# LoganWilliams1/mhm2_kmer_analysis_v2

Hardware: AMD Instinct MI355X
Metric: k-mers/sec (kcount stage) at k=21 (higher is better)
Workload: dtype u64

## Files before the change

### mhm2_kmer_analysis_v2_amd/csrc/kc_api.hip

```cpp
#include <hip/hip_runtime.h>

#include <math.h>
#include <stdio.h>
#include <stdlib.h>
#include <string.h>

#include <algorithm>
#include <new>
#include <thread>
#include <type_traits>
#include <vector>

#include "../../include/kcount_mi355.h"
#include "kc_bucketed.hpp"
#include "kc_shard.hpp"
#include "kc_wire6.hpp"
#include "kc_supermer.hpp"
#include "kc_ctg.hpp"

using namespace kc;

static thread_local char g_last_error[512] = "";

static int hip_fail(hipError_t e, const char *what, int line) {
// ... 630 lines not shown
  int rc = KC_OK;
  for (int i = 0; i < NCAND && !rc; i++) {
    rate[i] = probe(cand[i], wpw);
    const double gib = probe(cand[i], wpw_gib);
    if (rate[i] < 0 || gib <= 0) rc = KC_ERR_HIP;
    else ratio[i] = rate[i] / gib;
    if (log) fprintf(stderr, "kc arena probe (%s): allocation %d, %.2f TB/s, %.2f of its first GiB alone, %p\n", what, i, rate[i], ratio[i], (void *)cand[i]);
    if (rc || ratio[i] >= KC_ARENA_OK || i == NCAND - 1) break;
    size_t free_b = 0, total_b = 0;
    if (hipMemGetInfo(&free_b, &total_b) != hipSuccess || free_b < bytes + ((size_t)8 << 30)) break;
    if (hipMalloc((void **)&cand[i + 1], bytes) != hipSuccess) {
      (void)hipGetLastError();
      cand[i + 1] = nullptr;
      break;
    }
    ncand = i + 2;
  }
  int best_i = -1;
  for (int i = 0; i < ncand; i++)
    if (cand[i] && (best_i < 0 || ratio[i] > ratio[best_i])) best_i = i;
  for (int i = 0; i < ncand; i++)
    if (i != best_i && cand[i]) (void)hipFree(cand[i]);
  *arena = best_i >= 0 ? cand[best_i] : nullptr;
  c->arena_probe_tbps = best_i >= 0 ? rate[best_i] : 0.0;
  (void)hipEventDestroy(e0);
  (void)hipEventDestroy(e1);
  if (!rc && !*arena) rc = KC_ERR_OUT_OF_MEMORY;
  if (rc) snprintf(g_last_error, sizeof(g_last_error), "choosing the %s arena failed", what);
  return rc;
}

constexpr double KC_MAX_REGION_LOAD = 0.72;

static int bk_init(kc_ctx *c) {
  if (c->bk_ready) return KC_OK;
  const kc_tuning &t = c->tuning;
  Geom &g = c->gm;
  memset(&g, 0, sizeof(g));
  const uint64_t bcap = c->cfg.max_kmers_buffered ? c->cfg.max_kmers_buffered : (1ULL << 26);
  double est = c->cfg.max_elems ? (double)c->cfg.max_elems : 0.35 * (double)bcap;
  const double flow_n = ((c->cfg.flags & KC_FLAG_SHARD_BUCKETS) && c->cfg.rank_n > 1) ? (double)c->cfg.rank_n : 1.0;
  est *= flow_n;
  const uint32_t smax = count_smax(c->nl);
  g.S = t.slots ? std::min(std::max(t.slots, 16u), smax) : smax;
  while (g.S & (g.S - 1)) g.S &= g.S - 1;
  const double target_load = 0.4;
  if (!t.slots && est <= KC_MAX_REGION_LOAD * (double)(1u << 20) * (g.S / 2)) g.S /= 2;
  const uint64_t regions_needed = std::min<uint64_t>((uint64_t)(est / (target_load * g.S)) + 1, 1ULL << 20);
  g.P1 = t.p1 ? t.p1 : (uint32_t)std::max<double>(1.0, floor(sqrt((double)regions_needed)));
  g.P2 = t.p2 ? t.p2 : (uint32_t)((regions_needed + g.P1 - 1) / g.P1);
  if (c->nl == 1 && c->k <= KC_COMPACT_MAX_K && t.mode != 2) {
    uint32_t la = 0, lb = 0;
    if (t.p1 || t.p2) {
      la = ilog2(g.P1);
      lb = ilog2(g.P2);
    } else {
      const uint32_t lr = std::min<uint32_t>(20, ilog2(regions_needed));
      la = lr / 2;
      lb = lr - la;
      if (2u * (uint32_t)c->k + 6u <= 32u + lr && la >= 1) {
        g.P1 = 1u << la;
        g.P2 = 1u << lb;
      }
    }
    if (g.P1 == (1u << la) && g.P2 == (1u << lb) && la >= 1 && lb >= 1 && 2u * (uint32_t)c->k + 6u <= 32u + la + lb &&
        2u * (uint32_t)c->k > la + lb) {
      g.cp = 1;
      g.la = la;
      g.lb = lb;
      g.k2 = 2u * (uint32_t)c->k;
    }
  }
  if (g.P1 < 1 || g.P2 < 1 || g.P1 > PMAX || g.P2 > PMAX) return KC_ERR_INVALID_ARG;
  g.rec6 = (c->nl == 1 && g.cp && g.k2 - g.la <= 32) ? 1u : 0u;
  c->wire6 = (c->cfg.flags & KC_FLAG_WIRE_UNITS) && g.rec6 && g.k2 - g.la - g.lb >= 21 && !(c->cfg.flags & KC_FLAG_REFERENCE_OWNER) &&
             c->cfg.rank_n >= 1 && c->cfg.rank_n <= (int)WIRE6_MAX_SHARDS;
  g.G = t.writers ? std::min<uint32_t>(t.writers, GMAX)
                  : (uint32_t)std::max<uint64_t>(1, std::min<uint64_t>((uint64_t)std::min<int>(c->num_cus, GMAX), bcap / (4 * 16384)));
  if (g.G < 1) g.G = 1;
  const uint64_t R = (uint64_t)g.P1 * g.P2;
  const double mean1 = (double)bcap / ((double)g.G * g.P1), mean2 = flow_n * (double)bcap / (double)R;
  g.log2CH1 = t.chunk1 ? ilog2(t.chunk1) : std::min<uint32_t>(12, std::max<uint32_t>(4, ilog2((uint64_t)(mean1 / 8) + 1)));
  g.log2CH2 = t.chunk2 ? ilog2(t.chunk2) : std::min<uint32_t>(10, std::max<uint32_t>(4, ilog2((uint64_t)(mean2 / 8) + 1)));
  const uint64_t CH1 = 1ULL << g.log2CH1, CH2 = 1ULL << g.log2CH2;
  g.L1MAX = t.chain1_max ? t.chain1_max : (uint32_t)(4.0 * mean1 / (double)CH1) + 8;
  g.L2MAX = std::min<uint32_t>(CHAIN_LDS, t.chain2_max ? t.chain2_max : (uint32_t)(4.0 * mean2 / (double)CH2) + 8);
  if (g.cp && !t.chain2_max) g.L2MAX = std::min<uint32_t>(CHAIN_LDS, std::max<uint32_t>(g.L2MAX, (uint32_t)((KC_COUNT_MAX + CH2) / CH2) + 1));
  g.A1 = t.arena1 ? t.arena1 : (uint32_t)(1.03 * (double)bcap / ((double)g.G * (double)CH1)) + g.P1 + 16;
  const uint64_t a2 = bcap / CH2 + R + g.P1 + 16;
  if (a2 >= (1ULL << 32) || (uint64_t)g.A1 * g.G >= (1ULL << 32) || bcap / g.P1 >= (1ULL << 31)) return KC_ERR_INVALID_ARG;
  g.A2 = (uint32_t)a2;
  BucketBufs &b = c->bb;
  memset(&b, 0, sizeof(b));
  b.ovf1_cap = t.ovf_capacity ? t.ovf_capacity : std::max<uint64_t>(bcap / (c->nl == 1 ? 4 : 8) + 4096, 2 * (uint64_t)SUPER_SPAN);
  b.ovf2_cap = t.ovf_capacity ? t.ovf_capacity : std::max<uint64_t>(bcap / (c->nl == 1 ? 32 : 64) + 4096, 2 * (uint64_t)SUPER_SPAN);
  const size_t w = (size_t)c->nl * 8;
  const size_t nseg = (size_t)g.G * g.P1;
  const size_t rec1_bytes = (size_t)g.G * g.A1 * CH1 * (g.rec6 ? 6 : w) + 64, rec2_bytes = (size_t)g.A2 * CH2 * (g.cp ? 4 : w);
  bool rec1_reused = false, rec2_reused = false;
  {
    int rc = bk_take(c, 0, (void **)&b.rec1, rec1_bytes, &rec1_reused);
    const char *pe = getenv("KC_ARENA_PROBE");
    if (!rc && !(pe && pe[0] == '0') && rec1_bytes >= ((size_t)1 << 30) && !rec1_reused) {
      rc = pick_fast_arena(c, &b.rec1, rec1_bytes, g.G, "level 1");
    }
    if (!rc) rc = bk_take(c, 1, (void **)&b.chain1, nseg * g.L1MAX * 4);
    if (!rc) rc = bk_take(c, 2, (void **)&b.cnt1, nseg * 4);
    if (!rc) rc = bk_take(c, 3, (void **)&b.used1, (size_t)g.G * 2 * 4);
    if (!rc) rc = bk_take(c, 4, (void **)&b.rec2, rec2_bytes, &rec2_reused);
    if (!rc) rc = bk_take(c, 5, (void **)&b.chain2, (size_t)R * g.L2MAX * 4);
    if (!rc) rc = bk_take(c, 6, (void **)&b.cnt2, (size_t)R * 4);
    if (!rc) rc = bk_take(c, 7, (void **)&b.base2, ((size_t)g.P1 + 1) * 4);
    if (!rc) rc = bk_take(c, 8, (void **)&b.flag, (size_t)R * 4);
    if (!rc) rc = bk_take(c, 9, (void **)&b.ovf1, b.ovf1_cap * w);
    if (!rc) rc = bk_take(c, 10, (void **)&b.ovf2, b.ovf2_cap * w);
    if (!rc) rc = bk_take(c, 11, (void **)&b.done1, nseg * 4);
    if (!rc) rc = bk_take(c, 12, (void **)&b.used2, (size_t)g.P1 * 4);
    if (rc) return rc;
  }
  c->inc_on = false;
  c->l2_per_bucket = 0;
  HIPCHK(hipMemsetAsync(b.cnt1, 0, nseg * 4, c->stream));
  HIPCHK(hipMemsetAsync(b.used1, 0, (size_t)g.G * 2 * 4, c->stream));
  HIPCHK(hipMemsetAsync(b.cnt2, 0, (size_t)R * 4, c->stream));
  HIPCHK(hipMemsetAsync(b.flag, 0, (size_t)R * 4, c->stream));
  HIPCHK(hipMemsetAsync(c->d_cb, 0, CB_COUNT * 8, c->stream));
  if (getenv("KC_DEBUG_ADDR"))
    fprintf(stderr, "kc arenas: rec1 %p (%zu MB) chain1 %p cnt1 %p rec2 %p chain2 %p ovf1 %p ovf2 %p\n", (void *)b.rec1, rec1_bytes >> 20,
            (void *)b.chain1, (void *)b.cnt1, (void *)b.rec2, (void *)b.chain2, (void *)b.ovf1, (void *)b.ovf2);
  c->bk_bytes = rec1_bytes + rec2_bytes + (b.ovf1_cap + b.ovf2_cap) * w + nseg * (g.L1MAX + 1) * 4 + (size_t)R * (g.L2MAX + 2) * 4;
  c->bk_capacity = bcap;
  c->bk_ready = true;
  c->bk_level2 = c->bk_flagged = false;
  c->bk_rot = 0;
  return KC_OK;
}

static int sync_cb(kc_ctx *c) {
  HIPCHK(hipMemcpyAsync(c->h_cb, c->d_cb, CB_COUNT * 8, hipMemcpyDeviceToHost, c->stream));
  HIPCHK(hipStreamSynchronize(c->stream));
  return KC_OK;
}

static int bk_ovf1_room(kc_ctx *c, uint64_t want, uint64_t *room) {
  if (c->ovf1_ub + want <= c->bb.ovf1_cap) {
    *room = c->bb.ovf1_cap - c->ovf1_ub;
    return KC_OK;
  }
  int rc = sync_cb(c);
  if (rc) return rc;
  if (c->h_cb[CB_FATAL] & ~(c->inc_on ? (uint64_t)FATAL_OVF2 : 0ULL)) {
    snprintf(g_last_error, sizeof(g_last_error), "k-mer buffer: records were lost (fatal bits %llu)", (unsigned long long)c->h_cb[CB_FATAL]);
    return KC_ERR_CAPACITY;
  }
  uint64_t used = std::min<uint64_t>(c->h_cb[CB_OVF1], c->bb.ovf1_cap);
  if (used && c->bb.ovf1_cap - used < want && !c->sh.extracting) {
    rc = ensure_room(c, used);
    if (rc) return rc;
    {
      KernelTimer kt(c, KT_FALLBACK);
      with_nl(c, [&](auto nl) {
        auto kern = with_cp<nl>(c, [&](auto cp) { return kc_ovf1_drain_kernel<nl, cp>; });
        hipLaunchKernelGGL(kern, dim3((unsigned)std::min<uint64_t>((used + TPB - 1) / TPB, 256 * 32)), dim3(TPB), 0, c->stream, c->gm, c->bb,
                           used, c->table, c->d_ctrs);
      });
    }
// ... 1297 lines not shown
  *owner = (int)shard_of_bucket(b1, c->gm.P1, (uint32_t)c->cfg.rank_n);
  return KC_OK;
}

extern "C" int kc_flush(kc_ctx *c) {
  if (!c) return KC_ERR_INVALID_ARG;
  HIPCHK(hipSetDevice(c->cfg.device));
  int rc = sync_ctrs(c);
  if (rc) return rc;
  if (c->h_ctrs[CTR_BAD_BASE]) return KC_ERR_BAD_BASE;
  return KC_OK;
}

static int alloc_results(kc_ctx *c, uint64_t cap) {
  if (!cap) cap = 1;
  if (c->d_out_keys && c->out_cap >= cap) {
    c->out_n = 0;
    free_index(c);
    return KC_OK;
  }
  free_results(c);
  HIPCHK(hipMalloc((void **)&c->d_out_keys, cap * c->nl * 8));
  HIPCHK(hipMalloc((void **)&c->d_out_counts, cap * 2));
  HIPCHK(hipMalloc((void **)&c->d_out_left, cap));
  HIPCHK(hipMalloc((void **)&c->d_out_right, cap));
  c->out_cap = cap;
  return KC_OK;
}

static int grow_results(kc_ctx *c, uint64_t need, uint64_t keep) {
  if (need <= c->out_cap) return KC_OK;
  uint64_t *k0 = c->d_out_keys;
  uint16_t *c0 = c->d_out_counts;
  uint8_t *l0 = c->d_out_left, *r0 = c->d_out_right;
  c->d_out_keys = nullptr;
  c->d_out_counts = nullptr;
  c->d_out_left = c->d_out_right = nullptr;
  int rc = alloc_results(c, need);
  if (!rc && keep) {
    HIPCHK(hipMemcpyAsync(c->d_out_keys, k0, keep * c->nl * 8, hipMemcpyDeviceToDevice, c->stream));
    HIPCHK(hipMemcpyAsync(c->d_out_counts, c0, keep * 2, hipMemcpyDeviceToDevice, c->stream));
    HIPCHK(hipMemcpyAsync(c->d_out_left, l0, keep, hipMemcpyDeviceToDevice, c->stream));
    HIPCHK(hipMemcpyAsync(c->d_out_right, r0, keep, hipMemcpyDeviceToDevice, c->stream));
    HIPCHK(hipStreamSynchronize(c->stream));
  }
  if (k0) (void)hipFree(k0);
  if (c0) (void)hipFree(c0);
  if (l0) (void)hipFree(l0);
  if (r0) (void)hipFree(r0);
  return rc;
}

static int table_finalize_append(kc_ctx *c) {
  int rc = sync_ctrs(c);
  if (rc) return rc;
  const uint64_t entries = c->h_ctrs[CTR_ENTRIES];
  if (!entries) return KC_OK;
  rc = grow_results(c, c->h_ctrs[CTR_OUT] + entries, c->h_ctrs[CTR_OUT]);
  if (rc) return rc;
  {
    KernelTimer kt(c, KT_FINALIZE);
    const unsigned nblk = (unsigned)std::min<uint64_t>((c->capacity + TPB - 1) / TPB, 256 * 16);
    with_nl(c, [&](auto nl) {
      hipLaunchKernelGGL(kc_finalize_kernel<nl>, dim3(nblk), dim3(TPB), 0, c->stream, c->table, c->capacity, c->cfg.dmin_thres, c->d_out_keys,
                         c->d_out_counts, c->d_out_left, c->d_out_right, c->d_ctrs);
    });
  }
  HIPCHK(hipGetLastError());
  return KC_OK;
}

template <int NL>
static int bk_level2_launch(kc_ctx *c, bool inc) {
  const bool cr = use_cp<NL>(c) && c->gm.k2 - c->gm.la <= 32;
  const bool fl = shard_flow_only(c);
  if (inc && fl) return KC_ERR_STATE;
  auto kern = with_cp<NL>(c, [&](auto cp) {
    if (inc) return cr ? kc_l2_split_kernel<NL, cp, cp, false, true> : kc_l2_split_kernel<NL, cp, false, false, true>;
    if (cr) return fl ? kc_l2_split_kernel<NL, cp, cp, true> : kc_l2_split_kernel<NL, cp, cp, false>;
    return fl ? kc_l2_split_kernel<NL, cp, false, true> : kc_l2_split_kernel<NL, cp, false, false>;
  });
  const bool r6 = NL == 1 && c->gm.rec6 != 0;
  auto kern6 = inc ? kc_l2_rec6_kernel<false, true> : (fl ? kc_l2_rec6_kernel<true, false> : kc_l2_rec6_kernel<false, false>);
  int rc = r6 ? set_dyn_lds(kern6, l2r6_lds_bytes()) : set_dyn_lds(kern, lds_l2<NL>());
  if (rc) return rc;
  FlatSrc fs;
  memset(&fs, 0, sizeof(fs));
  fs.b_hi = c->gm.P1;
  if (fl) {
    fs.cnt = c->sh.d_cnt;
    fs.at = c->sh.d_at;
    fs.F = c->sh.F;
    fs.b_lo = shard_first_bucket((uint32_t)c->cfg.rank_me, c->gm.P1, (uint32_t)c->cfg.rank_n);
    fs.b_hi = shard_first_bucket((uint32_t)c->cfg.rank_me + 1, c->gm.P1, (uint32_t)c->cfg.rank_n);
    fs.nbo = fs.b_hi - fs.b_lo;
  }
  if (!inc || !c->inc_on) {
    if (inc && !c->l2_per_bucket) c->l2_per_bucket = (c->bk_capacity + c->gm.P1 - 1) / c->gm.P1;
    const uint64_t per_bucket = inc ? c->l2_per_bucket : 0;
    hipLaunchKernelGGL(kc_bucket_prefix_kernel, dim3(1), dim3(WGB), 0, c->stream, c->gm, c->bb, fs, c->d_cb, per_bucket);
    c->num_gpu_calls++;
    if (inc) {
      HIPCHK(hipMemsetAsync(c->bb.cnt2, 0, (size_t)c->gm.P1 * c->gm.P2 * 4, c->stream));
      HIPCHK(hipMemsetAsync(c->bb.done1, 0, (size_t)c->gm.G * c->gm.P1 * 4, c->stream));
      HIPCHK(hipMemsetAsync(c->bb.used2, 0, (size_t)c->gm.P1 * 4, c->stream));
      c->inc_on = true;
    }
  }
  if (fs.b_hi > fs.b_lo) {
    KernelTimer kt(c, r6 ? KT_L2_REC6 : KT_L2_SPLIT);
    const dim3 grid(std::min<unsigned>(fs.b_hi - fs.b_lo, (unsigned)c->num_cus));
    if (r6) hipLaunchKernelGGL(kern6, grid, dim3(WGB), l2r6_lds_bytes(), c->stream, c->gm, c->bb, fs, c->d_cb);
    else hipLaunchKernelGGL(kern, grid, dim3(WGB), lds_l2<NL>(), c->stream, c->gm, c->bb, fs, c->d_cb);
  }
  HIPCHK(hipGetLastError());
  return KC_OK;
}

static int bk_level2_instalment(kc_ctx *c) {
  if (!bk_active(c) || !c->bk_ready || c->bk_level2 || c->sh.flow) return KC_OK;
  return with_nl(c, [&](auto nl) { return bk_level2_launch<nl>(c, true); });
}

static int bk_l2_reserve(kc_ctx *c, uint64_t need) {
  const Geom &g = c->gm;
  const uint64_t CH2 = 1ULL << g.log2CH2;
  const uint64_t pb_need = (uint64_t)((double)need * 1.08 / (double)g.P1) + 2 * CH2;
  const uint64_t pb_now = c->inc_on ? c->l2_per_bucket : (c->bk_capacity + g.P1 - 1) / g.P1;
  if (pb_need <= pb_now) {
    if (!c->inc_on) c->l2_per_bucket = pb_now;
    return KC_OK;
  }
  const uint64_t pb = c->inc_on ? std::max<uint64_t>(2 * pb_now, pb_need) : pb_need;
  const uint64_t a2 = (uint64_t)g.P1 * ((pb + CH2 - 1) / CH2 + g.P2) + 16;
  if (a2 >= (1ULL << 32)) return KC_ERR_OUT_OF_MEMORY;
  uint64_t *bigger = nullptr;
  const size_t bytes = (size_t)a2 * CH2 * 4;
  size_t free_b = 0, total_b = 0;
  if (hipMemGetInfo(&free_b, &total_b) != hipSuccess || free_b < bytes + ((size_t)4 << 30) || hipMalloc((void **)&bigger, bytes) != hipSuccess) {
    (void)hipGetLastError();
    return KC_ERR_OUT_OF_MEMORY;
  }
  if (c->inc_on) {
    uint32_t *nb = nullptr;
    if (hipMalloc((void **)&nb, ((size_t)g.P1 + 1) * 4) != hipSuccess) {
      (void)hipGetLastError();
      (void)hipFree(bigger);
      return KC_ERR_OUT_OF_MEMORY;
    }
    BucketBufs tmp = c->bb;
    tmp.base2 = nb;
    FlatSrc fs;
    memset(&fs, 0, sizeof(fs));
    hipLaunchKernelGGL(kc_bucket_prefix_kernel, dim3(1), dim3(WGB), 0, c->stream, c->gm, tmp, fs, c->d_cb, pb);
    hipLaunchKernelGGL(kc_l2_grow_kernel, dim3(g.P1), dim3(WGB), 0, c->stream, c->gm, reinterpret_cast<const uint32_t *>(c->bb.rec2),
                       reinterpret_cast<uint32_t *>(bigger), c->bb.base2, nb, c->bb.used2, c->bb.chain2, c->bb.cnt2);
    c->num_gpu_calls += 2;
    hipError_t e = hipGetLastError();
    if (e == hipSuccess) e = hipMemcpyAsync(c->bb.base2, nb, ((size_t)g.P1 + 1) * 4, hipMemcpyDeviceToDevice, c->stream);
    if (e == hipSuccess) e = hipStreamSynchronize(c->stream);
    (void)hipFree(nb);
    if (e != hipSuccess) {
      (void)hipFree(bigger);
      return hip_fail(e, "bk_l2_reserve", __LINE__);
    }
  }
  HIPCHK(hipFree(c->bb.rec2));
  c->bk_bytes += bytes - c->bk_held[4];
  c->bb.rec2 = bigger;
  c->bk_held[4] = bytes;
  c->gm.A2 = (uint32_t)a2;
  c->l2_per_bucket = pb;
  return KC_OK;
}

static int l2_snapshot(kc_ctx *c) {
  const Geom &g = c->gm;
  const size_t b_cnt2 = (size_t)g.P1 * g.P2 * 4, b_used2 = (size_t)g.P1 * 4, b_done1 = (size_t)g.G * g.P1 * 4, need = b_cnt2 + b_used2 + b_done1 + 8;
  c->l2snap_fresh = !c->inc_on;
  if (c->l2snap_fresh) return KC_OK;
  if (c->l2snap_bytes < need) {
    if (c->d_l2snap) HIPCHK(hipFree(c->d_l2snap));
    c->d_l2snap = nullptr;
    c->l2snap_bytes = 0;
    HIPCHK(hipMalloc((void **)&c->d_l2snap, need));
    c->l2snap_bytes = need;
  }
  HIPCHK(hipMemcpyAsync(c->d_l2snap, c->bb.cnt2, b_cnt2, hipMemcpyDeviceToDevice, c->stream));
  HIPCHK(hipMemcpyAsync(c->d_l2snap + b_cnt2, c->bb.used2, b_used2, hipMemcpyDeviceToDevice, c->stream));
  HIPCHK(hipMemcpyAsync(c->d_l2snap + b_cnt2 + b_used2, c->bb.done1, b_done1, hipMemcpyDeviceToDevice, c->stream));
  HIPCHK(hipMemcpyAsync(c->d_l2snap + b_cnt2 + b_used2 + b_done1, c->d_cb + CB_OVF2, 8, hipMemcpyDeviceToDevice, c->stream));
  return KC_OK;
}
static int l2_restore_and_grow(kc_ctx *c, uint64_t need, uint64_t kept) {
  const Geom &g = c->gm;
// ... 925 lines not shown
```

### mhm2_kmer_analysis_v2_amd/csrc/kc_bucketed.hpp

```cpp
#pragma once
#include "kc_kernels.hpp"

namespace kc {

constexpr int WGB = 1024;
constexpr int SUPER_SPAN = 16 * WGB - PRE - POST;
using TileSuper = TileGeo<WGB, SUPER_SPAN>;
static_assert(TileSuper::GPT == 1 && TileSuper::NGROUP == WGB, "one group per thread");
constexpr int PMAX = 1024;
constexpr int GMAX = 512;

template <int NL> struct Rnd {
  static constexpr int RPOS = NL == 1 ? 16 : NL == 2 ? 8 : 4;
  static constexpr int RPOS_READS = NL == 1 ? 8 : NL <= 3 ? 4 : 2;
  static constexpr size_t STAGE = ((size_t)WGB * RPOS + 64) * NL * 8;
  static constexpr size_t STAGE_READS = ((size_t)WGB * RPOS_READS + 64) * NL * 8;
};

struct Geom {
  uint32_t G, P1, P2, S;
  uint32_t log2CH1, log2CH2;
  uint32_t L1MAX, L2MAX;
  uint32_t A1;
  uint32_t A2;
// ... 1219 lines not shown
          } else {
            lo[j] = (uint32_t)(nxt[j][0] >> (64u - gm.k2));
            ext = (uint32_t)nxt[j][0] & 63u;
          }
          br[j] = ((lo[j] >> sh_b2) & (P2 - 1u)) | (ext << 10);
        } else {
#pragma unroll
          for (int w = 0; w < NL; w++) rec[j][w] = nxt[j][w];
        }
      }
    };
    if (n) load_round(0);
    take_over();
    if (per_round < n) load_round(per_round);
    int buf = 0;
    for (uint32_t v0 = 0; v0 < n; v0 += per_round) {
#pragma unroll
      for (int j = 0; j < RPOS; j++) {
        const bool valid = v0 + (uint32_t)j * WGB + tid < n;
        uint32_t b;
        if constexpr (CR) b = br[j] & (PMAX - 1);
        else b = CP ? cp_b2(rec[j][0], gm) : hash_b2(rec_hash<NL>(rec[j]), gm);
        const uint32_t rank = hist_rank(L.sp, buf, b, valid);
        if constexpr (CR) br[j] = valid ? (br[j] | (rank << 16)) : ~0u;
        else br[j] = valid ? (b | (rank << 10)) : ~0u;
      }
      KC_SPLIT_STAMP(0)
      lds_barrier();
      const uint32_t total = split_stage<NL, RPOS, CR ? 16 : 10>(
          L.sp, sorted, nullptr, buf, P2,
          [&](int j, uint64_t (&o)[NL]) {
            if constexpr (CR) {
              o[0] = ((uint64_t)b1 << (64u - gm.la)) | ((uint64_t)lo[j] << (64u - gm.k2)) | (uint64_t)((br[j] >> 10) & 63u);
            } else {
#pragma unroll
              for (int w = 0; w < NL; w++) o[w] = rec[j][w];
            }
          },
          br, D, cst);
      take_over();
      if (v0 + 2 * (uint64_t)per_round < n) load_round(v0 + 2 * per_round);
      KC_SPLIT_STAMP(5)
      split_copy_out<NL>(
          L.sp, sorted, nullptr, total, D, [&](const uint64_t (&r)[NL]) { return CP ? cp_b2(r[0], gm) : hash_b2(rec_hash<NL>(r), gm); },
          [&](uint32_t b, const uint64_t (&r)[NL]) {
            bb.flag[(size_t)b1 * P2 + b] = 1;
            const uint64_t o = atomicAdd((unsigned long long *)&cb[CB_OVF2], 1ULL);
            if (o < bb.ovf2_cap) {
#pragma unroll
              for (int w = 0; w < NL; w++) bb.ovf2[o * NL + w] = (CP && w == 0) ? cp_unmix_rec(r[w], gm) : r[w];
            } else {
              atomicOr((unsigned long long *)&cb[CB_FATAL], (unsigned long long)FATAL_OVF2);
            }
          },
          [&](size_t i, const uint64_t (&r)[NL]) {
            if (CP) reinterpret_cast<uint32_t *>(D.arena)[i] = cp_pack32(r[0], gm);
            else store_words<NL>(D.arena, i, r);
          });
      buf ^= 1;
    }
    {
      const int tid = fresh_tid();
      if ((uint32_t)tid < P2) bb.cnt2[(size_t)b1 * P2 + tid] = cst.cur;
      if constexpr (INC) {
        if ((uint32_t)tid < G) bb.done1[(size_t)tid * P1 + b1] = L.skip[tid] + (L.pre[tid + 1] - L.pre[tid]);
        if (tid == 0) bb.used2[b1] = min(L.sp.arena_used, D.arena_cap);
      }
    }
    __syncthreads();
  }
}

struct L2R6LDS {
  SplitLDS sp;
  uint32_t pre[GMAX + 1];
  uint32_t end[GMAX];
  union {
    uint64_t flo[FLAT_MAX];
    uint32_t skip[GMAX];
  };
};
constexpr size_t l2r6_lds_bytes() { return ((sizeof(L2R6LDS) + 15) & ~size_t(15)) + Rnd<1>::STAGE; }
static_assert(l2r6_lds_bytes() <= 160 * 1024, "level 2's working set fits the LDS");
struct __attribute__((packed, aligned(2))) Load12 {
  uint32_t a, b, c;
};

template <bool FL, bool INC>
__global__ __launch_bounds__(WGB) void kc_l2_rec6_kernel(Geom gm, BucketBufs bb, FlatSrc fs, uint64_t *cb) {
  static_assert(!(INC && FL), "instalments are for a context that is not in the shard flow");
  extern __shared__ __align__(16) uint8_t smem[];
  L2R6LDS &L = *reinterpret_cast<L2R6LDS *>(smem);
  uint64_t *sorted = reinterpret_cast<uint64_t *>(smem + ((sizeof(L2R6LDS) + 15) & ~size_t(15)));
  constexpr int RPOS = 16, NPAIR = 8;
  const int tid = threadIdx.x;
  const uint32_t P1 = gm.P1, P2 = gm.P2, G = gm.G;
  const uint32_t GT = FL ? G + fs.F : G;
  const uint32_t CH1m = (1u << gm.log2CH1) - 1u;
  const uint8_t *const rec1 = reinterpret_cast<const uint8_t *>(bb.rec1);
  for (uint32_t b1 = (FL ? fs.b_lo : 0u) + blockIdx.x; b1 < (FL ? fs.b_hi : P1); b1 += gridDim.x) {
    {
      const int tid = fresh_tid();
      uint32_t v = 0;
      if ((uint32_t)tid < G) {
        const uint32_t cnt = bb.cnt1[(size_t)tid * P1 + b1];
        uint32_t d = 0;
        if constexpr (INC) {
          d = bb.done1[(size_t)tid * P1 + b1];
          L.skip[tid] = d;
        }
        L.end[tid] = cnt;
        v = cnt > d ? ((cnt - (d & ~1u) + 1u) & ~1u) : 0u;
      }
      if constexpr (FL) {
        if ((uint32_t)tid >= G && (uint32_t)tid < GT) {
          const uint32_t c = fs.cnt[(size_t)(tid - G) * fs.nbo + (b1 - fs.b_lo)];
          L.flo[tid - G] = fs.at[(size_t)(tid - G) * fs.nbo + (b1 - fs.b_lo)];
          L.end[tid] = c;
          v = (c + 1u) & ~1u;
        }
      }
      const uint32_t e = block_excl_scan(v, L.sp.scan);
      if ((uint32_t)tid < GT) L.pre[tid] = e;
      if (tid == 0) L.pre[GT] = L.sp.scan.total;
    }
    ChainDest D;
    D.arena = bb.rec2;
    D.chain = bb.chain2 + (size_t)b1 * P2 * gm.L2MAX;
    D.log2CH = gm.log2CH2;
    D.LMAX = gm.L2MAX;
    D.arena_base = bb.base2[b1];
    D.arena_cap = bb.base2[b1 + 1] - bb.base2[b1];
    D.own_lo = 0;
    D.own_hi = PMAX;
#ifdef KC_STAMPS
    unsigned long long tprev_ = __builtin_amdgcn_s_memtime();
    D.stamps = cb + 8;
    D.tprev = &tprev_;
#endif
    ChainState cst = split_load_state(L.sp, P2, INC ? bb.cnt2 + (size_t)b1 * P2 : nullptr, D.chain, D.LMAX, D.log2CH, INC ? bb.used2[b1] : 0u);
    __syncthreads();
    const uint32_t n = L.pre[GT];
    const uint32_t per_round = WGB * RPOS;
    uint32_t p_ids = 0, p_rec = 0;
    Load12 nxt[NPAIR];
    uint32_t nxt_valid = 0, nxt_flat = 0;
    auto load_round = [&](uint32_t v0) {
      uint32_t ids[NPAIR];
#pragma unroll
      for (int j = 0; j < NPAIR; j++) {
        const uint32_t e = min(v0 + 2u * ((uint32_t)j * WGB + tid), n - 2u);
        while (e >= L.pre[p_ids + 1]) p_ids++;
        const uint32_t i0 = e - L.pre[p_ids] + (INC ? (L.skip[p_ids] & ~1u) : 0u);
        const size_t ci = ((size_t)p_ids * gm.P1 + b1) * gm.L1MAX + (i0 >> gm.log2CH1);
        ids[j] = bb.chain1[FL && p_ids >= G ? 0 : ci];
      }
      nxt_valid = 0;
#pragma unroll
      for (int j = 0; j < NPAIR; j++) {
        const uint32_t ev = v0 + 2u * ((uint32_t)j * WGB + tid), e = min(ev, n - 2u);
        while (e >= L.pre[p_rec + 1]) p_rec++;
        const bool flat = FL && p_rec >= G;
        const uint32_t first = (INC && !flat) ? L.skip[p_rec] : 0u;
        const uint32_t i0 = e - L.pre[p_rec] + (first & ~1u), end = L.end[p_rec];
        const uint8_t *src = rec1 + ((((size_t)p_rec * gm.A1 + ids[j]) << gm.log2CH1) + (i0 & CH1m)) * 6;
        if constexpr (FL) {
          const uint64_t f0 = L.flo[flat ? p_rec - G : 0u];
          if (flat) src = reinterpret_cast<const uint8_t *>((uintptr_t)f0) + 5u * (size_t)i0;
          nxt_flat = flat ? (nxt_flat | (1u << j)) : (nxt_flat & ~(1u << j));
        }
        const bool in = ev < n;
        nxt_valid |= (in && i0 >= first && i0 < end ? 1u : 0u) << (2 * j);
        nxt_valid |= (in && i0 + 1u < end ? 2u : 0u) << (2 * j);
        nxt[j] = *reinterpret_cast<const Load12 *>(src);
      }
    };
    uint32_t lo[RPOS], br[RPOS];
    uint32_t cur_valid = 0;
    const uint32_t sh_b2 = gm.k2 - gm.la - gm.lb;
    auto take_over = [&]() {
#pragma unroll
      for (int j = 0; j < NPAIR; j++) {
        const Load12 w = nxt[j];
        uint32_t e0, e1;
        if (FL && ((nxt_flat >> j) & 1u)) {
          lo[2 * j] = w.a;
          e0 = w.b & 63u;
          lo[2 * j + 1] = (w.b >> 8) | (w.c << 24);
          e1 = (w.c >> 8) & 63u;
        } else {
          lo[2 * j] = w.a;
          e0 = (w.b >> 10) & 63u;
          lo[2 * j + 1] = (w.b >> 16) | (w.c << 16);
          e1 = w.c >> 26;
        }
        br[2 * j] = ((lo[2 * j] >> sh_b2) & (P2 - 1u)) | (e0 << 10);
        br[2 * j + 1] = ((lo[2 * j + 1] >> sh_b2) & (P2 - 1u)) | (e1 << 10);
      }
      cur_valid = nxt_valid;
    };
    if (n) load_round(0);
    take_over();
    if (per_round < n) load_round(per_round);
    int buf = 0;
    for (uint32_t v0 = 0; v0 < n; v0 += per_round) {
#pragma unroll
      for (int j = 0; j < RPOS; j++) {
        const bool valid = (cur_valid >> j) & 1u;
        const uint32_t rank = hist_rank(L.sp, buf, br[j] & (PMAX - 1), valid);
        br[j] = valid ? (br[j] | (rank << 16)) : ~0u;
      }
      KC_SPLIT_STAMP(0)
      lds_barrier();
      const uint32_t total = split_stage<1, RPOS, 16>(
          L.sp, sorted, nullptr, buf, P2,
          [&](int j, uint64_t (&o)[1]) {
            o[0] = ((uint64_t)b1 << (64u - gm.la)) | ((uint64_t)lo[j] << (64u - gm.k2)) | (uint64_t)((br[j] >> 10) & 63u);
          },
          br, D, cst);
      take_over();
      if (v0 + 2 * (uint64_t)per_round < n) load_round(v0 + 2 * per_round);
      KC_SPLIT_STAMP(5)
      split_copy_out<1>(
          L.sp, sorted, nullptr, total, D, [&](const uint64_t (&r)[1]) { return cp_b2(r[0], gm); },
          [&](uint32_t b, const uint64_t (&r)[1]) {
            bb.flag[(size_t)b1 * P2 + b] = 1;
            const uint64_t o = atomicAdd((unsigned long long *)&cb[CB_OVF2], 1ULL);
            if (o < bb.ovf2_cap) bb.ovf2[o] = cp_unmix_rec(r[0], gm);
            else atomicOr((unsigned long long *)&cb[CB_FATAL], (unsigned long long)FATAL_OVF2);
          },
          [&](size_t i, const uint64_t (&r)[1]) { reinterpret_cast<uint32_t *>(D.arena)[i] = cp_pack32(r[0], gm); });
      buf ^= 1;
    }
    {
      const int tid = fresh_tid();
      if ((uint32_t)tid < P2) bb.cnt2[(size_t)b1 * P2 + tid] = cst.cur;
      if constexpr (INC) {
        if ((uint32_t)tid < G) bb.done1[(size_t)tid * P1 + b1] = L.end[tid];
        if (tid == 0) bb.used2[b1] = min(L.sp.arena_used, D.arena_cap);
      }
    }
    __syncthreads();
  }
}

template <int NL, bool CP>
__global__ void kc_ovf1_to_regions_kernel(Geom gm, BucketBufs bb, uint64_t n, uint64_t *cb) {
  const uint64_t i = (uint64_t)blockIdx.x * blockDim.x + threadIdx.x;
  if (i >= n) return;
  uint64_t r[NL];
  for (int w = 0; w < NL; w++) r[w] = bb.ovf1[i * NL + w];
  size_t reg;
  if (CP) {
    const uint64_t m = cp_mix_rec(r[0], gm);
    reg = (size_t)cp_b1(m, gm) * gm.P2 + cp_b2(m, gm);
  } else {
    const uint64_t h = rec_hash<NL>(r);
    reg = (size_t)hash_b1(h, gm) * gm.P2 + hash_b2(h, gm);
  }
  bb.flag[reg] = 1;
  const uint64_t o = atomicAdd((unsigned long long *)&cb[CB_OVF2], 1ULL);
  if (o < bb.ovf2_cap) {
    for (int w = 0; w < NL; w++) bb.ovf2[o * NL + w] = r[w];
  } else {
    atomicOr((unsigned long long *)&cb[CB_FATAL], (unsigned long long)FATAL_OVF2);
  }
}

template <int NL, bool CP>
__global__ __launch_bounds__(TPB) void kc_ovf1_drain_kernel(Geom gm, BucketBufs bb, uint64_t n, Table t, uint64_t *ctrs) {
  for (uint64_t i = (uint64_t)blockIdx.x * TPB + threadIdx.x; i < n; i += (uint64_t)gridDim.x * TPB) {
    uint64_t r[NL];
    for (int w = 0; w < NL; w++) r[w] = bb.ovf1[i * NL + w];
    size_t reg;
    if (CP) {
      const uint64_t m = cp_mix_rec(r[0], gm);
      reg = (size_t)cp_b1(m, gm) * gm.P2 + cp_b2(m, gm);
    } else {
      const uint64_t h = rec_hash<NL>(r);
      reg = (size_t)hash_b1(h, gm) * gm.P2 + hash_b2(h, gm);
    }
    bb.flag[reg] = 1;
    table_insert<NL>(t, r, ctrs);
  }
}

constexpr uint32_t CHAIN_LDS = 480;

template <int NL>
struct CountLDS {
  static constexpr uint32_t SMAX = NL <= 2 ? 4096 : 2048;
  static constexpr int ew(bool) { return NL == 1 ? 6 : 5; }
  uint32_t chain[2][CHAIN_LDS];
  uint32_t hdr[2][2];
  uint32_t nout;
  uint32_t ncand;
  uint32_t fail[2];
  uint32_t gbase_lo, gbase_hi, gbase2_lo, gbase2_hi, split;
  static constexpr size_t header_bytes() { return (sizeof(CountLDS<NL>) + 15) & ~size_t(15); }
  static constexpr size_t bytes(uint32_t S, bool cp) { return header_bytes() + (size_t)S * ((cp ? 4 : 8 * NL) + 4 * ew(cp) + 2) + 16; }
};
static_assert(2 * CountLDS<2>::bytes(2048, false) <= 160 * 1024, "two workgroups of the two-word count kernel per CU");

struct CountTab {
  uint64_t *keys;
  uint32_t *ext;
  uint16_t *cand;
  uint32_t S, lgS;
};

template <int NL, bool CP>
__device__ __forceinline__ CountTab count_tab(uint8_t *smem, uint32_t S) {
  CountTab t;
  uint8_t *p = smem + CountLDS<NL>::header_bytes();
  t.keys = reinterpret_cast<uint64_t *>(p);
// ... 701 lines not shown
```

Measured before the change: 95.60 billion.

## Carry partial 16-record tails across rounds in level-2 rec6 split

In the non-incremental, non-flow rec6 level-2 kernel, each round now stages packed 32-bit records in LDS and writes only whole groups of 16 per bucket to the arena. Leftover records (up to 15 per bucket) are held in an LDS carry buffer and flushed at the end. The goal is aligned, coalesced 16-wide global writes in place of ragged per-round tails and the generic split_stage path. In exchange it uses more LDS, which may lower occupancy, and it forces a minimum chunk size of 16 for rec6.

Result: no change. 95.26 billion, median of 6 (-0.4%).

```diff
diff --git a/mhm2_kmer_analysis_v2_amd/csrc/kc_api.hip b/mhm2_kmer_analysis_v2_amd/csrc/kc_api.hip
--- a/mhm2_kmer_analysis_v2_amd/csrc/kc_api.hip
+++ b/mhm2_kmer_analysis_v2_amd/csrc/kc_api.hip
@@ -736,6 +736,7 @@
   const double mean1 = (double)bcap / ((double)g.G * g.P1), mean2 = flow_n * (double)bcap / (double)R;
   g.log2CH1 = t.chunk1 ? ilog2(t.chunk1) : std::min<uint32_t>(12, std::max<uint32_t>(4, ilog2((uint64_t)(mean1 / 8) + 1)));
   g.log2CH2 = t.chunk2 ? ilog2(t.chunk2) : std::min<uint32_t>(10, std::max<uint32_t>(4, ilog2((uint64_t)(mean2 / 8) + 1)));
+  if (g.rec6 && g.log2CH2 < 4) g.log2CH2 = 4;
   const uint64_t CH1 = 1ULL << g.log2CH1, CH2 = 1ULL << g.log2CH2;
   g.L1MAX = t.chain1_max ? t.chain1_max : (uint32_t)(4.0 * mean1 / (double)CH1) + 8;
   g.L2MAX = std::min<uint32_t>(CHAIN_LDS, t.chain2_max ? t.chain2_max : (uint32_t)(4.0 * mean2 / (double)CH2) + 8);
@@ -2199,7 +2200,8 @@
   });
   const bool r6 = NL == 1 && c->gm.rec6 != 0;
   auto kern6 = inc ? kc_l2_rec6_kernel<false, true> : (fl ? kc_l2_rec6_kernel<true, false> : kc_l2_rec6_kernel<false, false>);
-  int rc = r6 ? set_dyn_lds(kern6, l2r6_lds_bytes()) : set_dyn_lds(kern, lds_l2<NL>());
+  const size_t lds6 = inc || fl ? l2r6_lds_bytes() : l2r6_carry_lds_bytes();
+  int rc = r6 ? set_dyn_lds(kern6, lds6) : set_dyn_lds(kern, lds_l2<NL>());
   if (rc) return rc;
   FlatSrc fs;
   memset(&fs, 0, sizeof(fs));
@@ -2227,7 +2229,7 @@
   if (fs.b_hi > fs.b_lo) {
     KernelTimer kt(c, r6 ? KT_L2_REC6 : KT_L2_SPLIT);
     const dim3 grid(std::min<unsigned>(fs.b_hi - fs.b_lo, (unsigned)c->num_cus));
-    if (r6) hipLaunchKernelGGL(kern6, grid, dim3(WGB), l2r6_lds_bytes(), c->stream, c->gm, c->bb, fs, c->d_cb);
+    if (r6) hipLaunchKernelGGL(kern6, grid, dim3(WGB), lds6, c->stream, c->gm, c->bb, fs, c->d_cb);
     else hipLaunchKernelGGL(kern, grid, dim3(WGB), lds_l2<NL>(), c->stream, c->gm, c->bb, fs, c->d_cb);
   }
   HIPCHK(hipGetLastError());
diff --git a/mhm2_kmer_analysis_v2_amd/csrc/kc_bucketed.hpp b/mhm2_kmer_analysis_v2_amd/csrc/kc_bucketed.hpp
--- a/mhm2_kmer_analysis_v2_amd/csrc/kc_bucketed.hpp
+++ b/mhm2_kmer_analysis_v2_amd/csrc/kc_bucketed.hpp
@@ -1325,6 +1325,80 @@
 };
 constexpr size_t l2r6_lds_bytes() { return ((sizeof(L2R6LDS) + 15) & ~size_t(15)) + Rnd<1>::STAGE; }
 static_assert(l2r6_lds_bytes() <= 160 * 1024, "level 2's working set fits the LDS");
+
+constexpr uint32_t CARRY_MAX = 15;
+constexpr uint32_t C2_SLOTS = 16 * WGB + 64;
+constexpr size_t l2r6_carry_lds_bytes() {
+  return ((sizeof(L2R6LDS) + 15) & ~size_t(15)) + (size_t)C2_SLOTS * 4 + (size_t)PMAX * CARRY_MAX * 4;
+}
+static_assert(l2r6_carry_lds_bytes() <= 160 * 1024, "level 2's working set with the carry fits the LDS");
+
+__device__ __forceinline__ uint32_t carry_reserve(SplitLDS &L, int buf, uint32_t P, const ChainDest &D, ChainState &st, uint32_t &cc,
+                                                  bool flush) {
+  const int tid = fresh_tid();
+  const uint32_t v = ((uint32_t)tid < P) ? L.hist[buf][tid] : 0u;
+  const uint32_t excl = block_excl_scan(v, L.scan);
+  const uint32_t CHm = (1u << D.log2CH) - 1u;
+  if ((uint32_t)tid < P) {
+    const uint32_t base = st.cur, T = cc + v, out = flush ? T : (T & ~15u);
+    uint32_t fit = out;
+    const uint64_t room = ((uint64_t)D.LMAX << D.log2CH) - base;
+    if ((uint64_t)fit > room) fit = (uint32_t)room;
+    const uint32_t have = (base + CHm) >> D.log2CH;
+    uint32_t k = ((base + fit + CHm) >> D.log2CH) - have, a = 0;
+    if (k) {
+      a = atomicAdd(&L.arena_used, k);
+      const uint32_t left = D.arena_cap - min(D.arena_cap, L.arena_top);
+      if (a + k > left) {
+        k = a < left ? left - a : 0;
+        const uint64_t cap = ((uint64_t)(have + k) << D.log2CH) - base;
+        if ((uint64_t)fit > cap) fit = (uint32_t)cap;
+      }
+      uint32_t *ch = D.chain + (size_t)tid * D.LMAX + have;
+      for (uint32_t i = 0; i < k; i++) ch[i] = D.arena_base + a + i;
+    }
+    const uint32_t w = (base & CHm) ? min(fit, (CHm + 1u) - (base & CHm)) : 0u;
+    const bool ovf = fit < out;
+    uint4 d;
+    d.x = ((st.last - D.arena_base) << D.log2CH) + (base & CHm);
+    d.y = ((a - have) << D.log2CH) + base;
+    d.z = excl | (cc << 15) | (((w + 15u) >> 4) << 19) | (ovf ? 1u << 30 : 0u);
+    d.w = T | (fit << 16);
+    L.dst[tid] = d;
+    if (k) st.last = D.arena_base + a + k - 1;
+    st.cur = base + fit;
+    cc = ovf ? 0u : T - out;
+    L.hist[buf][tid] = excl;
+    L.hist[buf ^ 1][tid] = 0;
+  }
+  lds_barrier();
+  return L.scan.total;
+}
+
+template <class OvfFn>
+__device__ __forceinline__ void carry_copy_out(SplitLDS &L, const uint32_t *stg, uint32_t *carry, uint32_t P, const ChainDest &D,
+                                               OvfFn overflow) {
+  const int tid = fresh_tid();
+  const uint32_t l = (uint32_t)tid & 15u, r0 = ((uint32_t)tid >> 4) * 16u;
+  uint32_t *const arena = reinterpret_cast<uint32_t *>(D.arena) + ((size_t)D.arena_base << D.log2CH);
+  for (uint32_t r = r0; r < min(r0 + 16u, P); r++) {
+    const uint4 d = L.dst[r];
+    const uint32_t T = d.w & 0xFFFFu, fit = d.w >> 16, s = d.z & 0x7FFFu, c = (d.z >> 15) & 15u, wb = (d.z >> 19) & 0x7FFu;
+    const bool ovf = (d.z >> 30) & 1u;
+    uint32_t *const cr = carry + r * CARRY_MAX;
+    for (uint32_t e0 = 0; e0 < T; e0 += 16) {
+      const uint32_t e = e0 + l;
+      const uint32_t val = e < c ? cr[e] : stg[s + e - c];
+      if (e < fit) {
+        arena[(size_t)(((e0 >> 4) < wb ? d.x : d.y) + e)] = val;
+      } else if (e < T) {
+        if (ovf) overflow(r, val);
+        else cr[e - fit] = val;
+      }
+    }
+  }
+  KC_SPLIT_STAMP(4)
+}
 struct __attribute__((packed, aligned(2))) Load12 {
   uint32_t a, b, c;
 };
@@ -1333,8 +1407,10 @@
 __global__ __launch_bounds__(WGB) void kc_l2_rec6_kernel(Geom gm, BucketBufs bb, FlatSrc fs, uint64_t *cb) {
   static_assert(!(INC && FL), "instalments are for a context that is not in the shard flow");
   extern __shared__ __align__(16) uint8_t smem[];
+  constexpr bool CA = !FL && !INC;
   L2R6LDS &L = *reinterpret_cast<L2R6LDS *>(smem);
   uint64_t *sorted = reinterpret_cast<uint64_t *>(smem + ((sizeof(L2R6LDS) + 15) & ~size_t(15)));
+  uint32_t *const stg32 = reinterpret_cast<uint32_t *>(sorted), *const carry = stg32 + C2_SLOTS;
   constexpr int RPOS = 16, NPAIR = 8;
   const int tid = threadIdx.x;
   const uint32_t P1 = gm.P1, P2 = gm.P2, G = gm.G;
@@ -1382,6 +1458,7 @@
     D.tprev = &tprev_;
 #endif
     ChainState cst = split_load_state(L.sp, P2, INC ? bb.cnt2 + (size_t)b1 * P2 : nullptr, D.chain, D.LMAX, D.log2CH, INC ? bb.used2[b1] : 0u);
+    uint32_t cc = 0;
     __syncthreads();
     const uint32_t n = L.pre[GT];
     const uint32_t per_round = WGB * RPOS;
@@ -1442,6 +1519,12 @@
       }
       cur_valid = nxt_valid;
     };
+    const auto ovf2 = [&](uint32_t b, uint32_t rec32) {
+      bb.flag[(size_t)b1 * P2 + b] = 1;
+      const uint64_t o = atomicAdd((unsigned long long *)&cb[CB_OVF2], 1ULL);
+      if (o < bb.ovf2_cap) bb.ovf2[o] = cp_unpack_rec(rec32, (size_t)b1 * P2 + b, gm);
+      else atomicOr((unsigned long long *)&cb[CB_FATAL], (unsigned long long)FATAL_OVF2);
+    };
     if (n) load_round(0);
     take_over();
     if (per_round < n) load_round(per_round);
@@ -1455,6 +1538,31 @@
       }
       KC_SPLIT_STAMP(0)
       lds_barrier();
+      if constexpr (CA) {
+        carry_reserve(L.sp, buf, P2, D, cst, cc, false);
+        KC_SPLIT_STAMP(2)
+        const uint32_t rbm = (1u << sh_b2) - 1u;
+#pragma unroll
+        for (int j0 = 0; j0 < RPOS; j0 += 8) {
+          uint32_t pos[8];
+#pragma unroll
+          for (int j = 0; j < 8; j++) pos[j] = L.sp.hist[buf][br[j0 + j] & (PMAX - 1)];
+#pragma unroll
+          for (int j = 0; j < 8; j++) {
+            const uint32_t bj = br[j0 + j];
+            const uint32_t p = bj != ~0u ? pos[j] + (bj >> 16) : (uint32_t)(RPOS * WGB) + lane_id();
+            stg32[p] = ((lo[j0 + j] & rbm) << 6) | ((bj >> 10) & 63u);
+          }
+        }
+        lds_barrier();
+        KC_SPLIT_STAMP(3)
+        take_over();
+        if (v0 + 2 * (uint64_t)per_round < n) load_round(v0 + 2 * per_round);
+        KC_SPLIT_STAMP(5)
+        carry_copy_out(L.sp, stg32, carry, P2, D, ovf2);
+        buf ^= 1;
+        continue;
+      }
       const uint32_t total = split_stage<1, RPOS, 16>(
           L.sp, sorted, nullptr, buf, P2,
           [&](int j, uint64_t (&o)[1]) {
@@ -1474,6 +1582,11 @@
           },
           [&](size_t i, const uint64_t (&r)[1]) { reinterpret_cast<uint32_t *>(D.arena)[i] = cp_pack32(r[0], gm); });
       buf ^= 1;
+    }
+    if constexpr (CA) {
+      lds_barrier();
+      carry_reserve(L.sp, buf, P2, D, cst, cc, true);
+      carry_copy_out(L.sp, stg32, carry, P2, D, ovf2);
     }
     {
       const int tid = fresh_tid();
```
